# microsoft/MoGe

Measured on NVIDIA H100. Metric: images/sec ViT-L 518px fp16 (MoGe-2 infer), higher is better.
Workload: dtype fp16

## Files before the change

### moge_b200/csrc/common.cuh

```cuda
#pragma once
#include <cuda.h>
#include <cuda_runtime.h>
#include <cuda_fp16.h>
#include <cuda_bf16.h>
#include <stdint.h>
#include <stdio.h>
#include "wgmma.cuh"

namespace mg {

__device__ __forceinline__ uint32_t smem_u32(const void* p) {
    return static_cast<uint32_t>(__cvta_generic_to_shared(p));
}
__device__ __forceinline__ uint32_t lane_id() { return threadIdx.x & 31; }
__device__ __forceinline__ bool elect_one() {
    uint32_t pred;
    asm volatile(
        "{\n\t.reg .pred p;\n\t"
        "elect.sync _|p, 0xffffffff;\n\t"
        "selp.u32 %0, 1, 0, p;\n\t}"
        : "=r"(pred));
    return pred != 0;
}

__device__ __forceinline__ void pdl_launch_dependents() { asm volatile("griddepcontrol.launch_dependents;" ::: "memory"); }
__device__ __forceinline__ void pdl_wait() { asm volatile("griddepcontrol.wait;" ::: "memory"); }
__device__ __forceinline__ void pdl_prologue() {
    pdl_launch_dependents();
    pdl_wait();
}

__device__ __forceinline__ void mbar_init(uint64_t* bar, uint32_t count) {
    asm volatile("mbarrier.init.shared::cta.b64 [%0], %1;" ::"r"(smem_u32(bar)), "r"(count) : "memory");
}
__device__ __forceinline__ void fence_mbar_init() {
    asm volatile("fence.mbarrier_init.release.cluster;" ::: "memory");
}
__device__ __forceinline__ void fence_proxy_async_smem() {
    asm volatile("fence.proxy.async.shared::cta;" ::: "memory");
}
__device__ __forceinline__ void mbar_arrive_expect_tx(uint64_t* bar, uint32_t bytes) {
    asm volatile("mbarrier.arrive.expect_tx.shared::cta.b64 _, [%0], %1;" ::"r"(smem_u32(bar)), "r"(bytes) : "memory");
}
__device__ __forceinline__ void mbar_arrive(uint64_t* bar) {
    asm volatile("mbarrier.arrive.shared::cta.b64 _, [%0];" ::"r"(smem_u32(bar)) : "memory");
}
__device__ __forceinline__ bool mbar_try_wait(uint64_t* bar, uint32_t parity) {
    uint32_t ok;
    asm volatile(
        "{\n\t.reg .pred p;\n\t"
        "mbarrier.try_wait.parity.shared::cta.b64 p, [%1], %2;\n\t"
        "selp.u32 %0, 1, 0, p;\n\t}"
        : "=r"(ok)
        : "r"(smem_u32(bar)), "r"(parity)
        : "memory");
    return ok != 0;
}
#ifndef MG_WATCHDOG_SPINS
#define MG_WATCHDOG_SPINS (1u << 21)
#endif
constexpr int kMaxDynSmem = 232448;
__device__ __forceinline__ void mbar_wait(uint64_t* bar, uint32_t parity) {
    uint32_t spins = 0;
    while (!mbar_try_wait(bar, parity)) {
        if (++spins > MG_WATCHDOG_SPINS) __trap();
    }
}

__device__ __forceinline__ void tma_prefetch_desc(const CUtensorMap* m) {
    asm volatile("prefetch.tensormap [%0];" ::"l"(reinterpret_cast<uint64_t>(m)) : "memory");
}
__device__ __forceinline__ void tma_load_2d(void* dst, const CUtensorMap* m, uint64_t* bar, int c0, int c1) {
    asm volatile(
        "cp.async.bulk.tensor.2d.shared::cluster.global.mbarrier::complete_tx::bytes [%0], [%1, {%3, %4}], [%2];"
        ::"r"(smem_u32(dst)), "l"(reinterpret_cast<uint64_t>(m)), "r"(smem_u32(bar)), "r"(c0), "r"(c1)
        : "memory");
}
__device__ __forceinline__ void tma_load_3d(void* dst, const CUtensorMap* m, uint64_t* bar, int c0, int c1, int c2) {
    asm volatile(
        "cp.async.bulk.tensor.3d.shared::cluster.global.mbarrier::complete_tx::bytes [%0], [%1, {%3, %4, %5}], [%2];"
        ::"r"(smem_u32(dst)), "l"(reinterpret_cast<uint64_t>(m)), "r"(smem_u32(bar)), "r"(c0), "r"(c1), "r"(c2)
        : "memory");
}
__device__ __forceinline__ void tma_load_4d(void* dst, const CUtensorMap* m, uint64_t* bar, int c0, int c1, int c2,
                                            int c3) {
    asm volatile(
        "cp.async.bulk.tensor.4d.shared::cluster.global.mbarrier::complete_tx::bytes [%0], [%1, {%3, %4, %5, %6}], [%2];"
        ::"r"(smem_u32(dst)), "l"(reinterpret_cast<uint64_t>(m)), "r"(smem_u32(bar)), "r"(c0), "r"(c1), "r"(c2),
        "r"(c3)
        : "memory");
}

__device__ __forceinline__ uint64_t make_sdesc_sw128(uint32_t smem_addr, uint32_t lbo_bytes = 16, uint32_t sbo_bytes = 1024) {
    uint64_t d = 0;
    d |= static_cast<uint64_t>((smem_addr & 0x3FFFF) >> 4);
    d |= static_cast<uint64_t>((lbo_bytes >> 4) & 0x3FFF) << 16;
    d |= static_cast<uint64_t>((sbo_bytes >> 4) & 0x3FFF) << 32;
    d |= static_cast<uint64_t>(1) << 62;
    return d;
}
__device__ __forceinline__ void wgmma_fence() { asm volatile("wgmma.fence.sync.aligned;" ::: "memory"); }
__device__ __forceinline__ void wgmma_commit() { asm volatile("wgmma.commit_group.sync.aligned;" ::: "memory"); }
template <int N> __device__ __forceinline__ void wgmma_wait() { asm volatile("wgmma.wait_group.sync.aligned %0;" ::"n"(N) : "memory"); }
template <int N> __device__ __forceinline__ void reg_fence(float (&r)[N]) {
#pragma unroll
    for (int i = 0; i < N; ++i) asm volatile("" : "+f"(r[i])::"memory");
}
__device__ __forceinline__ void named_sync(uint32_t id, uint32_t count) {
    asm volatile("bar.sync %0, %1;" ::"r"(id), "r"(count) : "memory");
}
template <uint32_t R> __device__ __forceinline__ void regs_dec() { asm volatile("setmaxnreg.dec.sync.aligned.u32 %0;" ::"n"(R)); }
template <uint32_t R> __device__ __forceinline__ void regs_inc() { asm volatile("setmaxnreg.inc.sync.aligned.u32 %0;" ::"n"(R)); }

__device__ __forceinline__ float2 ffma2(float2 a, float2 b, float2 c) { return make_float2(fmaf(a.x, b.x, c.x), fmaf(a.y, b.y, c.y)); }
__device__ __forceinline__ float2 fadd2(float2 a, float2 b) { return make_float2(a.x + b.x, a.y + b.y); }
__device__ __forceinline__ float2 fmul2(float2 a, float2 b) { return make_float2(a.x * b.x, a.y * b.y); }

__device__ __forceinline__ float fmax3(float a, float b, float c) {
    float r;
    asm("max.f32 %0, %1, %2, %3;" : "=f"(r) : "f"(a), "f"(b), "f"(c));
    return r;
}
__device__ __forceinline__ float ex2_approx(float x) {
    float r;
    asm("ex2.approx.ftz.f32 %0, %1;" : "=f"(r) : "f"(x));
    return r;
}

template <bool BF16> struct H16;
template <> struct H16<false> {
    using T = __half;
    using T2 = __half2;
    static __device__ __forceinline__ uint32_t pack(float a, float b) {
        __half2 h = __floats2half2_rn(a, b);
        return *reinterpret_cast<uint32_t*>(&h);
    }
    static __device__ __forceinline__ float2 unpack(uint32_t u) {
        return __half22float2(*reinterpret_cast<__half2*>(&u));
    }
    static __device__ __forceinline__ T from_float(float a) { return __float2half_rn(a); }
    static __device__ __forceinline__ float to_float(T a) { return __half2float(a); }
};
template <> struct H16<true> {
    using T = __nv_bfloat16;
    using T2 = __nv_bfloat162;
    static __device__ __forceinline__ uint32_t pack(float a, float b) {
        __nv_bfloat162 h = __floats2bfloat162_rn(a, b);
        return *reinterpret_cast<uint32_t*>(&h);
    }
    static __device__ __forceinline__ float2 unpack(uint32_t u) {
        return __bfloat1622float2(*reinterpret_cast<__nv_bfloat162*>(&u));
    }
    static __device__ __forceinline__ T from_float(float a) { return __float2bfloat16_rn(a); }
    static __device__ __forceinline__ float to_float(T a) { return __bfloat162float(a); }
};

__device__ __forceinline__ float warp_sum(float v) {
#pragma unroll
    for (int o = 16; o > 0; o >>= 1) v += __shfl_xor_sync(0xffffffffu, v, o);
    return v;
}
__device__ __forceinline__ float warp_max(float v) {
#pragma unroll
    for (int o = 16; o > 0; o >>= 1) v = fmaxf(v, __shfl_xor_sync(0xffffffffu, v, o));
    return v;
}

}
```

### moge_b200/csrc/umma_kernel.cuh

```cuda
#pragma once
#include "common.cuh"
#include <type_traits>

namespace mg {

enum : int { AMODE_ROWS = 0, AMODE_TILES = 1 };
enum : int {
    EPI_STORE16 = 0,
    EPI_GELU16 = 1,
    EPI_RESID = 2,
    EPI_PATCH = 3,
    EPI_DEC = 4,
    EPI_HEADOUT = 5,
    EPI_NECKOUT = 6,
};

enum : int { MODE_GEMM = 0, MODE_CONV64 = 1, MODE_CONVH = 2 };
constexpr int TILE_M = 128;
constexpr int TILE_K = 64;
constexpr int TILE_PW = 16;
constexpr int TILE_PH = 8;

struct UmmaParams {
    int M;
    int N;
    int ntaps;
    int kb_main;
    int kb_aux;
    int num_m_tiles, num_n_tiles;
    int B, H, W;
    int tiles_x, tiles_y;
    void* out0;
    void* out1;
    void* out2;
    int accum;
    const float* bias;
    const float* vec1;
    const float* vec2;
    const void* skip;
    int ldo;
    int T;
    int Ho, Wo, Hop, Wop;
    int shuffle;
    int ncomp;
    float su, sv;
    void* x16;
    float2* stats_out;
    const float* ln_rstd;
    int stats_ld;
};

template <int BN, int MODE = MODE_GEMM> struct UmmaCfg {
    static constexpr int kHaloBytes = 160 * 128;
    static constexpr int kABytes = (MODE == MODE_GEMM) ? TILE_M * 128 : kHaloBytes;
    static constexpr int kBBytes = (MODE == MODE_GEMM) ? BN * 128 : (MODE == MODE_CONVH) ? 3 * BN * 128 : 0;
    static constexpr int kStageBytes = kABytes + kBBytes;
    static constexpr int kResidentBytes = (MODE == MODE_CONV64) ? 10 * BN * 128 : 0;
    static constexpr int kChunks = (BN < 32) ? 1 : BN / 32;
    static constexpr int kAccBytes = TILE_M * kChunks * 32 * 4;
    static constexpr int kFixedBytes = kAccBytes + kResidentBytes + 1024  + 256 ;
    static constexpr int kFit = (kMaxDynSmem - kFixedBytes) / kStageBytes;
    static constexpr int kStages = kFit > 8 ? 8 : kFit;
    static constexpr int kEpiWarps = (BN >= 64) ? 8 : 4;
    static constexpr int kThreads = 384;
    static constexpr int kSmemBytes = kStages * kStageBytes + kFixedBytes;
    static constexpr int kColsPerWarp = (kEpiWarps == 8) ? BN / 2 : BN;
    static_assert(kStages >= 2, "umma_kernel: fewer than two ring stages fit beside the accumulator tile");
    static_assert(kSmemBytes <= kMaxDynSmem, "umma_kernel: stage ring + accumulator tile exceed the shared memory of one CTA");
    static_assert((2 * kStages + 1) * 8 <= 256, "umma_kernel: barrier block overflows its 256 bytes");
};

template <int BN>
__device__ __forceinline__ const float4* acc_block(const float4* stg, int quarter, int col) {
    return stg + (quarter * UmmaCfg<BN>::kChunks + (col >> 5)) * 256;
}
template <int BN>
__device__ __forceinline__ void acc_stage(float4* stg, const float* d, int g, int wl, int lane) {
    float* s = reinterpret_cast<float*>(stg);
#pragma unroll
    for (int i = 0; i < BN / 2; i += 2) {
        const int row = 64 * g + 16 * wl + (lane >> 2) + 8 * ((i >> 1) & 1);
        const int col = 8 * (i >> 2) + 2 * (lane & 3);
        const int rl = row & 31, q = (col & 31) >> 2;
        float* blk = s + ((row >> 5) * UmmaCfg<BN>::kChunks + (col >> 5)) * 1024;
        *reinterpret_cast<float2*>(blk + (rl * 8 + (q ^ (rl & 7))) * 4 + (col & 3)) = make_float2(d[i], d[i + 1]);
    }
}
template <int NQ>
__device__ __forceinline__ void acc_row(const float4* blk, int lane, float* v) {
#pragma unroll
    for (int q = 0; q < NQ; ++q) {
        const float4 t = blk[lane * 8 + (q ^ (lane & 7))];
        v[4 * q] = t.x; v[4 * q + 1] = t.y; v[4 * q + 2] = t.z; v[4 * q + 3] = t.w;
    }
}

__device__ __forceinline__ float gelu_erf(float x) {
    const float ax = fabsf(x);
    float q = fmaf(-4.804994387e-04f, ax, 7.133518346e-03f);
    q = fmaf(q, ax, -5.194617063e-02f);
    q = fmaf(q, ax, -4.598676562e-01f);
    q = fmaf(q, ax, -1.150842190e+00f);
    q = fmaf(q, ax, -3.041332639e-05f);
    const float t = ax * ex2_approx(q);
    return fmaf(-0.5f, t, fmaxf(x, 0.0f));
}

__device__ __forceinline__ float2 gelu_erf2(float2 x) {
    const float2 ab = make_float2(fabsf(x.x), fabsf(x.y));
    const float2 ax = ab;
    float2 q = ffma2(make_float2(-4.804994387e-04f, -4.804994387e-04f), ax, make_float2(7.133518346e-03f, 7.133518346e-03f));
    q = ffma2(q, ax, make_float2(-5.194617063e-02f, -5.194617063e-02f));
    q = ffma2(q, ax, make_float2(-4.598676562e-01f, -4.598676562e-01f));
    q = ffma2(q, ax, make_float2(-1.150842190e+00f, -1.150842190e+00f));
    q = ffma2(q, ax, make_float2(-3.041332639e-05f, -3.041332639e-05f));
    const float2 t = fmul2(ab, make_float2(ex2_approx(q.x), ex2_approx(q.y)));
    return ffma2(make_float2(-0.5f, -0.5f), t, make_float2(fmaxf(x.x, 0.0f), fmaxf(x.y, 0.0f)));
}

static __device__ __noinline__ void store_px_border8(uint8_t* base, int b, int Y, int X, int Ho, int Wo, int Hop, int Wop,
                                                 int ld, int c0, uint2 q) {
    uint8_t* centre = base + (((static_cast<size_t>(b) * Hop + Y + 1) * Wop + X + 1) * ld + c0) * 2;
    *reinterpret_cast<uint2*>(centre) = q;
    if (Y != 0 && Y != Ho - 1 && X != 0 && X != Wo - 1) return;
    const int dy0 = (Y == 0) ? -1 : 0, dy1 = (Y == Ho - 1) ? 1 : 0;
    const int dx0 = (X == 0) ? -1 : 0, dx1 = (X == Wo - 1) ? 1 : 0;
    const ptrdiff_t rowp = static_cast<ptrdiff_t>(Wop) * ld * 2, colp = static_cast<ptrdiff_t>(ld) * 2;
    for (int dy = dy0; dy <= dy1; ++dy)
        for (int dx = dx0; dx <= dx1; ++dx)
            if (dy != 0 || dx != 0) *reinterpret_cast<uint2*>(centre + dy * rowp + dx * colp) = q;
}

struct LnRows { float rs[8]; };
__device__ __forceinline__ void ln_load(const UmmaParams& p, int mt, int quarter, int lane, LnRows& r) {
    const int sub = lane >> 3;
#pragma unroll
    for (int i = 0; i < 8; ++i) {
        const long grow = static_cast<long>(mt) * TILE_M + quarter * 32 + 4 * i + sub;
        r.rs[i] = (grow < p.M) ? p.ln_rstd[grow] : 1.f;
    }
}

enum : int { DF_RAW = 1, DF_RELU = 2, DF_SKIP = 4, DF_UV = 8, DF_SHUFFLE = 16 };

static __device__ __noinline__ void store_px_border16(uint8_t* base, int b, int Y, int X, int Ho, int Wo, int Hop, int Wop,
                                                      int ld, int c0, uint4 q) {
    uint8_t* centre = base + (((static_cast<size_t>(b) * Hop + Y + 1) * Wop + X + 1) * ld + c0) * 2;
    const int dy0 = (Y == 0) ? -1 : 0, dy1 = (Y == Ho - 1) ? 1 : 0;
    const int dx0 = (X == 0) ? -1 : 0, dx1 = (X == Wo - 1) ? 1 : 0;
    const ptrdiff_t rowp = static_cast<ptrdiff_t>(Wop) * ld * 2, colp = static_cast<ptrdiff_t>(ld) * 2;
    for (int dy = dy0; dy <= dy1; ++dy)
        for (int dx = dx0; dx <= dx1; ++dx)
            if (dy != 0 || dx != 0) *reinterpret_cast<uint4*>(centre + dy * rowp + dx * colp) = q;
}

template <int BN, int COLS, int AMODE, bool BF16, int DF>
__device__ __forceinline__ void epilogue_dec16(const UmmaParams& p, int mt, int nt, const float4* stg, int quarter, int lane,
                                               int col_begin) {
    using H = H16<BF16>;
    const bool has_raw = (DF < 0) ? (p.out0 != nullptr) : ((DF & DF_RAW) != 0);
    const bool has_relu = (DF < 0) ? (p.out1 != nullptr) : ((DF & DF_RELU) != 0);
    const bool has_skip = (DF < 0) ? (p.skip != nullptr) : ((DF & DF_SKIP) != 0);
    const bool has_uv = (DF < 0) ? (p.vec1 != nullptr) : ((DF & DF_UV) != 0);
    const bool shuffle = (DF < 0) ? (p.shuffle != 0) : ((DF & DF_SHUFFLE) != 0);
    const int sub = lane >> 2;
    const int q8 = lane & 3;
    int tile_b = 0, tile_y0 = 0, tile_x0 = 0;
    if (AMODE == AMODE_TILES) {
        const int per_img = p.tiles_x * p.tiles_y;
        tile_b = mt / per_img;
        const int r = mt % per_img;
        tile_y0 = (r / p.tiles_x) * TILE_PH;
        tile_x0 = (r % p.tiles_x) * TILE_PW;
    }
    bool ok[4];
    int rb[4], ry[4], rx[4], eflags[4];
    size_t roff[4];
    const int sh = shuffle ? 2 : 1;
#pragma unroll
    for (int i = 0; i < 4; ++i) {
        const int rl = quarter * 32 + 8 * i + sub;
        if (AMODE == AMODE_ROWS) {
            const long grow = static_cast<long>(mt) * TILE_M + rl;
            ok[i] = grow < p.M;
            rb[i] = static_cast<int>(grow / p.T);
            const int t = static_cast<int>(grow % p.T);
            ry[i] = t / p.W; rx[i] = t % p.W;
        } else {
            rb[i] = tile_b;
            ry[i] = tile_y0 + rl / TILE_PW;
            rx[i] = tile_x0 + rl % TILE_PW;
            ok[i] = (ry[i] < p.H) && (rx[i] < p.W);
        }
        roff[i] = ((static_cast<size_t>(rb[i]) * p.Hop + sh * ry[i] + 1) * p.Wop + sh * rx[i] + 1) * p.ldo * 2;
        eflags[i] = (ry[i] == 0 ? 1 : 0) | (ry[i] == p.H - 1 ? 2 : 0) | (rx[i] == 0 ? 4 : 0) | (rx[i] == p.W - 1 ? 8 : 0);
    }
    const float inv_wo = 1.0f / static_cast<float>(p.Wo), inv_ho = 1.0f / static_cast<float>(p.Ho);
    bool interior;
    if (AMODE == AMODE_TILES) interior = tile_y0 > 0 && tile_x0 > 0 && tile_y0 + TILE_PH < p.H && tile_x0 + TILE_PW < p.W;
    else interior = false;
    const int ldo_shift = ((p.ldo & (p.ldo - 1)) == 0) ? (31 - __clz(p.ldo)) : -1;
    auto chunk = [&](int c, auto fast_tag) {
        constexpr bool FAST = decltype(fast_tag)::value;
        const float4* scr = acc_block<BN>(stg, quarter, col_begin + c);
        const int col = nt * BN + col_begin + c;
        int co = col + 8 * q8, qd = 0, qmask = 15;
        size_t qoff = 0;
        if (shuffle) {
            qd = (ldo_shift >= 0) ? (col >> ldo_shift) : (col / p.ldo);
            co -= qd * p.ldo;
            qoff = (static_cast<size_t>(qd >> 1) * p.Wop + (qd & 1)) * p.ldo * 2;
            qmask = ((qd >> 1) ? 2 : 1) | ((qd & 1) ? 8 : 4);
        }
        qoff += static_cast<size_t>(co) * 2;
        const float4 b0 = *reinterpret_cast<const float4*>(p.bias + co), b1 = *reinterpret_cast<const float4*>(p.bias + co + 4);
        float4 g0 = make_float4(0.f, 0.f, 0.f, 0.f), g1 = g0, h0 = g0, h1 = g0;
        if (has_uv) {
            g0 = *reinterpret_cast<const float4*>(p.vec1 + co); g1 = *reinterpret_cast<const float4*>(p.vec1 + co + 4);
            h0 = *reinterpret_cast<const float4*>(p.vec2 + co); h1 = *reinterpret_cast<const float4*>(p.vec2 + co + 4);
        }
        uint4 sk[4];
#pragma unroll
        for (int i = 0; i < 4; ++i) {
            sk[i] = make_uint4(0u, 0u, 0u, 0u);
            if (has_skip && (FAST || ok[i])) sk[i] = *reinterpret_cast<const uint4*>(static_cast<const uint8_t*>(p.skip) + roff[i] + qoff);
        }
        uint4 pk_raw[4], pk_relu[4];
        unsigned edge_rows = 0;
#pragma unroll
        for (int i = 0; i < 4; ++i) {
            const int rl = 8 * i + sub;
            float4 a0 = scr[rl * 8 + ((2 * q8) ^ (rl & 7))];
            float4 a1 = scr[rl * 8 + ((2 * q8 + 1) ^ (rl & 7))];
            if (!FAST && !ok[i]) continue;
            a0.x += b0.x; a0.y += b0.y; a0.z += b0.z; a0.w += b0.w;
            a1.x += b1.x; a1.y += b1.y; a1.z += b1.z; a1.w += b1.w;
            if (has_skip) {
                const float2 s0 = H::unpack(sk[i].x), s1 = H::unpack(sk[i].y), s2 = H::unpack(sk[i].z), s3 = H::unpack(sk[i].w);
                a0.x += s0.x; a0.y += s0.y; a0.z += s1.x; a0.w += s1.y;
                a1.x += s2.x; a1.y += s2.y; a1.z += s3.x; a1.w += s3.y;
            }
            if (has_uv) {
                const int X = sh * rx[i] + (qd & 1), Y = sh * ry[i] + (qd >> 1);
                const float uu = p.su * ((2 * X + 1) * inv_wo - 1.0f);
                const float vv = p.sv * ((2 * Y + 1) * inv_ho - 1.0f);
                a0.x += g0.x * uu + h0.x * vv; a0.y += g0.y * uu + h0.y * vv; a0.z += g0.z * uu + h0.z * vv; a0.w += g0.w * uu + h0.w * vv;
                a1.x += g1.x * uu + h1.x * vv; a1.y += g1.y * uu + h1.y * vv; a1.z += g1.z * uu + h1.z * vv; a1.w += g1.w * uu + h1.w * vv;
            }
            if (!FAST && (eflags[i] & qmask) != 0) edge_rows |= 1u << i;
            if (has_raw) {
                pk_raw[i] = make_uint4(H::pack(a0.x, a0.y), H::pack(a0.z, a0.w), H::pack(a1.x, a1.y), H::pack(a1.z, a1.w));
                *reinterpret_cast<uint4*>(static_cast<uint8_t*>(p.out0) + roff[i] + qoff) = pk_raw[i];
            }
            if (has_relu) {
                pk_relu[i] = make_uint4(H::pack(fmaxf(a0.x, 0.f), fmaxf(a0.y, 0.f)), H::pack(fmaxf(a0.z, 0.f), fmaxf(a0.w, 0.f)),
                                        H::pack(fmaxf(a1.x, 0.f), fmaxf(a1.y, 0.f)), H::pack(fmaxf(a1.z, 0.f), fmaxf(a1.w, 0.f)));
                *reinterpret_cast<uint4*>(static_cast<uint8_t*>(p.out1) + roff[i] + qoff) = pk_relu[i];
            }
        }
        if (!FAST && edge_rows != 0) {
#pragma unroll
            for (int i = 0; i < 4; ++i)
                if (edge_rows >> i & 1) {
                    const int X = sh * rx[i] + (qd & 1), Y = sh * ry[i] + (qd >> 1);
                    if (has_raw) store_px_border16(static_cast<uint8_t*>(p.out0), rb[i], Y, X, p.Ho, p.Wo, p.Hop, p.Wop, p.ldo, co, pk_raw[i]);
                    if (has_relu) store_px_border16(static_cast<uint8_t*>(p.out1), rb[i], Y, X, p.Ho, p.Wo, p.Hop, p.Wop, p.ldo, co, pk_relu[i]);
                }
        }
    };
    if (interior) {
#pragma unroll 1
        for (int c = 0; c < COLS; c += 32) chunk(c, std::true_type{});
    } else {
#pragma unroll 1
        for (int c = 0; c < COLS; c += 32) chunk(c, std::false_type{});
    }
}



template <int BN, int COLS, int AMODE, int EPI, bool BF16, int DF = -1>
__device__ __forceinline__ void epilogue_tile(const UmmaParams& p, int mt, int nt, const float4* stg, int quarter,
                                              int lane, int col_begin, bool ln_rows_on = false, LnRows lnr = LnRows{}) {
    using H = H16<BF16>;
    const bool has_raw = (DF < 0) ? (p.out0 != nullptr) : ((DF & DF_RAW) != 0);
    const bool has_relu = (DF < 0) ? (p.out1 != nullptr) : ((DF & DF_RELU) != 0);
    const bool has_skip = (DF < 0) ? (p.skip != nullptr) : ((DF & DF_SKIP) != 0);
    const bool has_uv = (DF < 0) ? (p.vec1 != nullptr) : ((DF & DF_UV) != 0);
    const bool shuffle = (DF < 0) ? (p.shuffle != 0) : ((DF & DF_SHUFFLE) != 0);
    if (EPI == EPI_DEC) {
        epilogue_dec16<BN, COLS, AMODE, BF16, DF>(p, mt, nt, stg, quarter, lane, col_begin);
        return;
    }
    const int row = quarter * 32 + lane;
    const int sub = lane >> 3;
    const int q4 = lane & 7;
    if (EPI == EPI_HEADOUT) {
        const int per_img = p.tiles_x * p.tiles_y;
        const int b = mt / per_img;
        const int r = mt % per_img;
        const int py = (r / p.tiles_x) * TILE_PH + row / TILE_PW;
        const int px = (r % p.tiles_x) * TILE_PW + row % TILE_PW;
        const bool valid = (py < p.H) && (px < p.W);
        float v[16];
        acc_row<4>(acc_block<BN>(stg, quarter, 0), lane, v);
        if (valid) {
#pragma unroll
            for (int ph = 0; ph < 4; ++ph) {
                const int Y = 2 * py + (ph >> 1), X = 2 * px + (ph & 1);
                float o[3];
#pragma unroll
                for (int k = 0; k < 3; ++k) o[k] = (k < p.ncomp) ? v[ph * p.ncomp + k] + p.bias[k] : 0.f;
                if (p.vec1 != nullptr) {
                    const uint4* src = reinterpret_cast<const uint4*>(
                        static_cast<const uint8_t*>(p.skip) + ((static_cast<size_t>(b) * p.Hop + Y + 1) * p.Wop + X + 1) * 64);
#pragma unroll
                    for (int q = 0; q < 4; ++q) {
                        const uint4 u = src[q];
                        const uint32_t w[4] = {u.x, u.y, u.z, u.w};
#pragma unroll
                        for (int e = 0; e < 4; ++e) {
                            const float2 f = H::unpack(w[e]);
                            const int c = q * 8 + e * 2;
#pragma unroll
                            for (int k = 0; k < 3; ++k)
                                if (k < p.ncomp) o[k] += p.vec1[k * 32 + c] * f.x + p.vec1[k * 32 + c + 1] * f.y;
                        }
                    }
                }
                const size_t pix = (static_cast<size_t>(b) * p.Ho + Y) * p.Wo + X;
                if (p.accum) {
                    if (p.ncomp == 1) o[0] += static_cast<const float*>(p.out0)[pix];
                    else { const float4 t = static_cast<const float4*>(p.out0)[pix]; o[0] += t.x; o[1] += t.y; o[2] += t.z; }
                }
                if (p.ncomp == 1) static_cast<float*>(p.out0)[pix] = o[0];
                else static_cast<float4*>(p.out0)[pix] = make_float4(o[0], o[1], o[2], 0.f);
            }
        }
        __syncwarp();
    } else if (EPI == EPI_NECKOUT) {
        const int per_img = p.tiles_x * p.tiles_y;
        const int b = mt / per_img;
        const int r = mt % per_img;
        const int py = (r / p.tiles_x) * TILE_PH + row / TILE_PW;
        const int px = (r % p.tiles_x) * TILE_PW + row % TILE_PW;
        const bool valid = (py < p.H) && (px < p.W);
        float v[32];
        acc_row<8>(acc_block<BN>(stg, quarter, 0), lane, v);
        if (valid) {
            float b8[8], gu[8], gv[8];
#pragma unroll
            for (int k = 0; k < 8; ++k) { b8[k] = p.bias[k]; gu[k] = p.vec1[k]; gv[k] = p.vec2[k]; }
            const float inv_wo = 1.0f / static_cast<float>(p.Wo), inv_ho = 1.0f / static_cast<float>(p.Ho);
#pragma unroll
            for (int ph = 0; ph < 4; ++ph) {
                const int Y = 2 * py + (ph >> 1), X = 2 * px + (ph & 1);
                const float uu = p.su * ((2 * X + 1) * inv_wo - 1.0f);
                const float vv = p.sv * ((2 * Y + 1) * inv_ho - 1.0f);
                float o[8];
#pragma unroll
                for (int k = 0; k < 8; ++k) o[k] = v[ph * 8 + k] + b8[k] + gu[k] * uu + gv[k] * vv;
                const size_t pix = (static_cast<size_t>(b) * p.Ho + Y) * p.Wo + X;
                if (p.out0) static_cast<float4*>(p.out0)[pix] = make_float4(o[0], o[1], o[2], 0.f);
                if (p.out1) static_cast<float4*>(p.out1)[pix] = make_float4(o[3], o[4], o[5], 0.f);
                if (p.out2) static_cast<float*>(p.out2)[pix] = o[6];
            }
        }
        __syncwarp();
    } else {
        int tile_b = 0, tile_y0 = 0, tile_x0 = 0;
        if (AMODE == AMODE_TILES) {
            const int per_img = p.tiles_x * p.tiles_y;
            tile_b = mt / per_img;
            const int r = mt % per_img;
            tile_y0 = (r / p.tiles_x) * TILE_PH;
            tile_x0 = (r % p.tiles_x) * TILE_PW;
        }
        bool ok[8];
        int rb[8], ry[8], rx[8];
        size_t roff[8];
        int eflags[8];
        int xrow[8];
#pragma unroll
        for (int i = 0; i < 8; ++i) {
            const int rl = quarter * 32 + 4 * i + sub;
            rb[i] = 0; ry[i] = 0; rx[i] = 0; roff[i] = 0; eflags[i] = 0; xrow[i] = 0;
            if (AMODE == AMODE_ROWS) {
                const long grow = static_cast<long>(mt) * TILE_M + rl;
                ok[i] = grow < p.M;
                xrow[i] = static_cast<int>(grow);
                roff[i] = static_cast<size_t>(grow) * p.ldo;
                if (EPI == EPI_DEC || EPI == EPI_PATCH) {
                    rb[i] = static_cast<int>(grow / p.T);
                    const int t = static_cast<int>(grow % p.T);
                    ry[i] = t / p.W; rx[i] = t % p.W;
                    if (EPI == EPI_PATCH) {
                        xrow[i] = rb[i] * (p.T + 1) + 1 + t;
                        roff[i] = static_cast<size_t>(xrow[i]) * p.ldo;
                    }
                }
            } else {
                rb[i] = tile_b;
                ry[i] = tile_y0 + rl / TILE_PW;
                rx[i] = tile_x0 + rl % TILE_PW;
                ok[i] = (ry[i] < p.H) && (rx[i] < p.W);
            }
            if (EPI == EPI_DEC) {
                const int sh = shuffle ? 2 : 1;
                roff[i] = ((static_cast<size_t>(rb[i]) * p.Hop + sh * ry[i] + 1) * p.Wop + sh * rx[i] + 1) * p.ldo * 2;
                eflags[i] = (ry[i] == 0 ? 1 : 0) | (ry[i] == p.H - 1 ? 2 : 0) | (rx[i] == 0 ? 4 : 0) | (rx[i] == p.W - 1 ? 8 : 0);
            }
        }
        const float inv_wo = 1.0f / static_cast<float>(p.Wo), inv_ho = 1.0f / static_cast<float>(p.Ho);
        constexpr bool LN_CONS = (EPI == EPI_STORE16 || EPI == EPI_GELU16) && AMODE == AMODE_ROWS;
        constexpr bool LN_PROD = (EPI == EPI_RESID || EPI == EPI_PATCH) && AMODE == AMODE_ROWS;
        const bool ln_on = LN_CONS && ln_rows_on;
        const bool x16_on = LN_PROD && p.x16 != nullptr;
        float ln_rs[8], st1[8], st2[8];
#pragma unroll
        for (int i = 0; i < 8; ++i) { ln_rs[i] = ln_on ? lnr.rs[i] : 1.f; st1[i] = 0.f; st2[i] = 0.f; }
        const bool full_tile = (AMODE == AMODE_ROWS) && (static_cast<long>(mt) + 1) * TILE_M <= static_cast<long>(p.M);
        auto chunk = [&](int c, auto full_tag) {
            constexpr bool FULL = decltype(full_tag)::value;
            const int col = nt * BN + col_begin + c;
            int co = col + 4 * q4;
            float4 pre[8];
            const float4* scr = acc_block<BN>(stg, quarter, col_begin + c);
            int qd = 0;
            size_t qoff = 0;
            int qmask = 15;
            if (EPI == EPI_DEC && shuffle) {
                qd = col / p.ldo;
                co -= qd * p.ldo;
                qoff = (static_cast<size_t>(qd >> 1) * p.Wop + (qd & 1)) * p.ldo * 2;
                qmask = ((qd >> 1) ? 2 : 1) | ((qd & 1) ? 8 : 4);
            }
            if (EPI == EPI_DEC) qoff += static_cast<size_t>(co) * 2;
            float4 bias4 = make_float4(0.f, 0.f, 0.f, 0.f), g4 = bias4, h4 = bias4;
            if (EPI != EPI_PATCH) bias4 = *reinterpret_cast<const float4*>(p.bias + co);
            if (EPI == EPI_RESID) g4 = *reinterpret_cast<const float4*>(p.vec1 + co);
            if (EPI == EPI_DEC && has_uv) {
                g4 = *reinterpret_cast<const float4*>(p.vec1 + co);
                h4 = *reinterpret_cast<const float4*>(p.vec2 + co);
            }
            int sY[8], sX[8];
#pragma unroll
            for (int i = 0; i < 8; ++i) {
                pre[i] = make_float4(0.f, 0.f, 0.f, 0.f);
                sY[i] = ry[i]; sX[i] = rx[i];
                if (EPI == EPI_DEC && shuffle) { sY[i] = 2 * ry[i] + (qd >> 1); sX[i] = 2 * rx[i] + (qd & 1); }
                if (!FULL && !ok[i]) continue;
                if (EPI == EPI_RESID) {
                    pre[i] = *reinterpret_cast<const float4*>(static_cast<const float*>(p.out0) + roff[i] + co);
                } else if (EPI == EPI_PATCH) {
                    const int t = ry[i] * p.W + rx[i];
                    pre[i] = *reinterpret_cast<const float4*>(p.vec1 + static_cast<size_t>(t) * p.ldo + co);
                } else if (EPI == EPI_DEC && has_skip) {
                    const uint2 u = *reinterpret_cast<const uint2*>(static_cast<const uint8_t*>(p.skip) + roff[i] + qoff);
                    const float2 f0 = H::unpack(u.x), f1 = H::unpack(u.y);
                    pre[i] = make_float4(f0.x, f0.y, f1.x, f1.y);
                }
            }
            uint2 pk_raw[8], pk_relu[8];
            unsigned edge_rows = 0;
#pragma unroll
            for (int i = 0; i < 8; ++i) {
                const int rl = 4 * i + sub;
                float4 a = scr[rl * 8 + (q4 ^ (rl & 7))];
                if (!FULL && !ok[i]) continue;
                if (EPI == EPI_STORE16 || EPI == EPI_GELU16) {
                    float2 a01, a23;
                    if (ln_on) {
                        a01 = make_float2(fmaf(ln_rs[i], a.x, bias4.x), fmaf(ln_rs[i], a.y, bias4.y));
                        a23 = make_float2(fmaf(ln_rs[i], a.z, bias4.z), fmaf(ln_rs[i], a.w, bias4.w));
                    } else {
                        a01 = make_float2(a.x + bias4.x, a.y + bias4.y);
                        a23 = make_float2(a.z + bias4.z, a.w + bias4.w);
                    }
                    if (EPI == EPI_GELU16) { a01 = gelu_erf2(a01); a23 = gelu_erf2(a23); }
                    uint2 pk;
                    pk.x = H::pack(a01.x, a01.y); pk.y = H::pack(a23.x, a23.y);
                    *reinterpret_cast<uint2*>(static_cast<typename H::T*>(p.out0) + roff[i] + co) = pk;
                } else if (EPI == EPI_RESID) {
                    float4 x = pre[i];
                    x.x += g4.x * (a.x + bias4.x); x.y += g4.y * (a.y + bias4.y);
                    x.z += g4.z * (a.z + bias4.z); x.w += g4.w * (a.w + bias4.w);
                    *reinterpret_cast<float4*>(static_cast<float*>(p.out0) + roff[i] + co) = x;
                    const float2 x01 = make_float2(x.x, x.y), x23 = make_float2(x.z, x.w);
                    if (x16_on) {
                        uint2 pk;
                        pk.x = H::pack(x01.x, x01.y); pk.y = H::pack(x23.x, x23.y);
                        *reinterpret_cast<uint2*>(static_cast<typename H::T*>(p.x16) + roff[i] + co) = pk;
                        const float2 f0 = H::unpack(pk.x), f1 = H::unpack(pk.y);
                        const float2 s1 = fadd2(f0, f1), s2 = ffma2(f0, f0, fmul2(f1, f1));
                        st1[i] += s1.x + s1.y;
                        st2[i] += s2.x + s2.y;
                    }
                } else if (EPI == EPI_PATCH) {
                    const float4 x = make_float4(a.x + pre[i].x, a.y + pre[i].y, a.z + pre[i].z, a.w + pre[i].w);
                    *reinterpret_cast<float4*>(static_cast<float*>(p.out0) + roff[i] + co) = x;
                    if (x16_on) {
                        uint2 pk;
                        pk.x = H::pack(x.x, x.y); pk.y = H::pack(x.z, x.w);
                        *reinterpret_cast<uint2*>(static_cast<typename H::T*>(p.x16) + roff[i] + co) = pk;
                        const float2 f0 = H::unpack(pk.x), f1 = H::unpack(pk.y);
                        const float2 s1 = fadd2(f0, f1), s2 = ffma2(f0, f0, fmul2(f1, f1));
                        st1[i] += s1.x + s1.y;
                        st2[i] += s2.x + s2.y;
                    }
                } else if (EPI == EPI_DEC) {
                    a.x += bias4.x + pre[i].x; a.y += bias4.y + pre[i].y; a.z += bias4.z + pre[i].z; a.w += bias4.w + pre[i].w;
                    if (has_uv) {
                        const float uu = p.su * ((2 * sX[i] + 1) * inv_wo - 1.0f);
                        const float vv = p.sv * ((2 * sY[i] + 1) * inv_ho - 1.0f);
                        a.x += g4.x * uu + h4.x * vv; a.y += g4.y * uu + h4.y * vv;
                        a.z += g4.z * uu + h4.z * vv; a.w += g4.w * uu + h4.w * vv;
                    }
                    if ((eflags[i] & qmask) != 0) edge_rows |= 1u << i;
                    if (has_raw) {
                        pk_raw[i].x = H::pack(a.x, a.y); pk_raw[i].y = H::pack(a.z, a.w);
                        *reinterpret_cast<uint2*>(static_cast<uint8_t*>(p.out0) + roff[i] + qoff) = pk_raw[i];
                    }
                    if (has_relu) {
                        pk_relu[i].x = H::pack(fmaxf(a.x, 0.f), fmaxf(a.y, 0.f)); pk_relu[i].y = H::pack(fmaxf(a.z, 0.f), fmaxf(a.w, 0.f));
                        *reinterpret_cast<uint2*>(static_cast<uint8_t*>(p.out1) + roff[i] + qoff) = pk_relu[i];
                    }
                }
            }
            if (EPI == EPI_DEC && edge_rows != 0) {
#pragma unroll
                for (int i = 0; i < 8; ++i)
                    if (edge_rows >> i & 1) {
                        if (has_raw) store_px_border8(static_cast<uint8_t*>(p.out0), rb[i], sY[i], sX[i], p.Ho, p.Wo, p.Hop, p.Wop, p.ldo, co, pk_raw[i]);
                        if (has_relu) store_px_border8(static_cast<uint8_t*>(p.out1), rb[i], sY[i], sX[i], p.Ho, p.Wo, p.Hop, p.Wop, p.ldo, co, pk_relu[i]);
                    }
            }
            __syncwarp();
        };
        if (full_tile) {
#pragma unroll 1
            for (int c = 0; c < COLS; c += 32) chunk(c, std::true_type{});
        } else {
#pragma unroll 1
            for (int c = 0; c < COLS; c += 32) chunk(c, std::false_type{});
        }
        if (x16_on) {
            const int part = (nt * BN + col_begin) / COLS;
#pragma unroll
            for (int i = 0; i < 8; ++i) {
                float a = st1[i], b = st2[i];
#pragma unroll
                for (int o = 1; o < 8; o <<= 1) { a += __shfl_xor_sync(0xffffffffu, a, o); b += __shfl_xor_sync(0xffffffffu, b, o); }
                if (q4 == 0 && ok[i]) p.stats_out[static_cast<size_t>(xrow[i]) * p.stats_ld + part] = make_float2(a, b);
            }
        }
    }
}

template <int BN, int MODE, int AMODE, int EPI, bool BF16, int DF = -1>
__global__ void __launch_bounds__(384, 1)
umma_kernel(const __grid_constant__ CUtensorMap mapA, const __grid_constant__ CUtensorMap mapAux,
            const __grid_constant__ CUtensorMap mapB, const UmmaParams p) {
    pdl_launch_dependents();
    using Cfg = UmmaCfg<BN, MODE>;
    constexpr int S = Cfg::kStages;
    extern __shared__ uint8_t smem_raw[];
    uint8_t* smem = smem_raw + ((1024u - (smem_u32(smem_raw) & 1023u)) & 1023u);
    float4* stg = reinterpret_cast<float4*>(smem + S * Cfg::kStageBytes);
    uint8_t* sW = smem + S * Cfg::kStageBytes + Cfg::kAccBytes;
    uint64_t* full = reinterpret_cast<uint64_t*>(sW + Cfg::kResidentBytes);
    uint64_t* empty = full + S;
    uint64_t* wfull = empty + S;

    const int warp = threadIdx.x >> 5;
    const int lane = threadIdx.x & 31;
    const int total_tiles = p.num_m_tiles * p.num_n_tiles;
    const int kb_taps = p.ntaps * p.kb_main;
    const int nstage = (MODE == MODE_GEMM) ? kb_taps + p.kb_aux : (MODE == MODE_CONV64) ? 3 + p.kb_aux : 3 * p.kb_main + p.kb_aux;

    if (threadIdx.x == 0) {
        tma_prefetch_desc(&mapA);
        tma_prefetch_desc(&mapB);
        if (p.kb_aux) tma_prefetch_desc(&mapAux);
        for (int s = 0; s < S; ++s) { mbar_init(&full[s], 1); mbar_init(&empty[s], 8); }
        mbar_init(wfull, 1);
        fence_mbar_init();
    }
    __syncthreads();
    pdl_wait();

    if (warp < 4) {
        regs_dec<40>();
        if (warp != 0) return;
        if (MODE == MODE_CONV64) {
            const int nblk = 9 + p.kb_aux;
            const int nt = static_cast<int>(blockIdx.x) % p.num_n_tiles;
            if (elect_one()) {
                mbar_arrive_expect_tx(wfull, nblk * BN * 128);
                for (int t = 0; t < nblk; ++t) tma_load_2d(sW + t * BN * 128, &mapB, wfull, t * TILE_K, nt * BN);
            }
            __syncwarp();
        }
        int s = 0; uint32_t ph = 0;
        for (int tile = blockIdx.x; tile < total_tiles; tile += gridDim.x) {
            const int mt = tile / p.num_n_tiles, nt = tile % p.num_n_tiles;
            int b = 0, x0 = 0, y0 = 0;
            if (AMODE == AMODE_TILES) {
                const int per_img = p.tiles_x * p.tiles_y;
                b = mt / per_img;
                const int r = mt % per_img;
                y0 = (r / p.tiles_x) * TILE_PH;
                x0 = (r % p.tiles_x) * TILE_PW;
            }
            for (int i = 0; i < nstage; ++i) {
                mbar_wait(&empty[s], ph ^ 1);
                uint8_t* sa = smem + s * Cfg::kStageBytes;
                uint8_t* sb = sa + Cfg::kABytes;
                if (elect_one()) {
                    if (MODE == MODE_GEMM) {
                        mbar_arrive_expect_tx(&full[s], Cfg::kStageBytes);
                        if (AMODE == AMODE_ROWS) {
                            tma_load_2d(sa, &mapA, &full[s], i * TILE_K, mt * TILE_M);
                        } else if (i < kb_taps) {
                            const int tap = i / p.kb_main, c = i % p.kb_main;
                            const int tx = (p.ntaps == 9) ? tap % 3 : 1, ty = (p.ntaps == 9) ? tap / 3 : 1;
                            tma_load_4d(sa, &mapA, &full[s], c * TILE_K, x0 + tx, y0 + ty, b);
                        } else {
                            tma_load_4d(sa, &mapAux, &full[s], (i - kb_taps) * TILE_K, x0 + 1, y0 + 1, b);
                        }
                        tma_load_2d(sb, &mapB, &full[s], i * TILE_K, nt * BN);
                    } else if (MODE == MODE_CONV64) {
                        if (i < 3) {
                            mbar_arrive_expect_tx(&full[s], Cfg::kHaloBytes);
                            tma_load_4d(sa, &mapA, &full[s], 0, x0 + i, y0, b);
                        } else {
                            mbar_arrive_expect_tx(&full[s], TILE_M * 128);
                            tma_load_4d(sa, &mapAux, &full[s], 0, x0 + 1, y0 + 1, b);
                        }
                    } else {
                        const bool aux = i >= 3 * p.kb_main;
                        if (!aux) {
                            const int c = i / 3, dx = i % 3;
                            mbar_arrive_expect_tx(&full[s], Cfg::kHaloBytes + 3 * BN * 128);
                            tma_load_4d(sa, &mapA, &full[s], c * TILE_K, x0 + dx, y0, b);
                            for (int dy = 0; dy < 3; ++dy)
                                tma_load_2d(sb + dy * BN * 128, &mapB, &full[s], ((dy * 3 + dx) * p.kb_main + c) * TILE_K, nt * BN);
                        } else {
                            const int c = i - 3 * p.kb_main;
                            mbar_arrive_expect_tx(&full[s], TILE_M * 128 + BN * 128);
                            tma_load_4d(sa, &mapAux, &full[s], c * TILE_K, x0 + 1, y0 + 1, b);
                            tma_load_2d(sb, &mapB, &full[s], (9 * p.kb_main + c) * TILE_K, nt * BN);
                        }
                    }
                }
                __syncwarp();
                if (++s == S) { s = 0; ph ^= 1; }
            }
        }
    } else {
        regs_inc<232>();
        const int g = (warp - 4) >> 2;
        const int wl = warp & 3;
        const int ew = warp - 4;
        const int quarter = ew & 3;
        const int col_begin = (Cfg::kEpiWarps == 8) ? (ew >> 2) * (BN / 2) : 0;
        const uint32_t a_off = static_cast<uint32_t>(g) * 64 * 128;
        if (MODE == MODE_CONV64) mbar_wait(wfull, 0);
        const uint32_t w0 = smem_u32(sW);
        LnRows lnr{}, lnn{};
        const bool ln_on = AMODE == AMODE_ROWS && (EPI == EPI_STORE16 || EPI == EPI_GELU16) && p.ln_rstd != nullptr;
        if (ln_on && static_cast<int>(blockIdx.x) < total_tiles) ln_load(p, static_cast<int>(blockIdx.x) / p.num_n_tiles, quarter, lane, lnn);
        int s = 0; uint32_t ph = 0;
        for (int tile = blockIdx.x; tile < total_tiles; tile += gridDim.x) {
            const int mt = tile / p.num_n_tiles, nt = tile % p.num_n_tiles;
            if (ln_on) {
                lnr = lnn;
                const int nxt = tile + static_cast<int>(gridDim.x);
                if (nxt < total_tiles) ln_load(p, nxt / p.num_n_tiles, quarter, lane, lnn);
            }
            float acc[BN / 2];
#pragma unroll
            for (int j = 0; j < BN / 2; ++j) acc[j] = 0.f;
            int prev = -1;
            for (int i = 0; i < nstage; ++i) {
                mbar_wait(&full[s], ph);
                const uint32_t sa = smem_u32(smem + s * Cfg::kStageBytes) + a_off;
                const uint32_t sb = smem_u32(smem + s * Cfg::kStageBytes + Cfg::kABytes);
                wgmma_fence();
                auto mma64 = [&](uint32_t a, uint32_t bb) {
                    const uint64_t ad = make_sdesc_sw128(a), bd = make_sdesc_sw128(bb);
#pragma unroll
                    for (int k = 0; k < TILE_K / 16; ++k) Wgmma<BN, BF16>::ss(acc, ad + 2 * k, bd + 2 * k, 1u);
                };
                if (MODE == MODE_GEMM) {
                    mma64(sa, sb);
                } else if (MODE == MODE_CONV64) {
                    if (i < 3) {
#pragma unroll
                        for (int dy = 0; dy < 3; ++dy) mma64(sa + dy * TILE_PW * 128, w0 + (dy * 3 + i) * BN * 128);
                    } else {
                        mma64(sa, w0 + 9 * BN * 128);
                    }
                } else {
                    if (i < 3 * p.kb_main) {
#pragma unroll
                        for (int dy = 0; dy < 3; ++dy) mma64(sa + dy * TILE_PW * 128, sb + dy * BN * 128);
                    } else {
                        mma64(sa, sb);
                    }
                }
                wgmma_commit();
                wgmma_wait<1>();
                reg_fence(acc);
                if (prev >= 0 && lane == 0) mbar_arrive(&empty[prev]);
                prev = s;
                if (++s == S) { s = 0; ph ^= 1; }
            }
            wgmma_wait<0>();
            reg_fence(acc);
            if (prev >= 0 && lane == 0) mbar_arrive(&empty[prev]);
            named_sync(1, 256);
            acc_stage<BN>(stg, acc, g, wl, lane);
            named_sync(1, 256);
            if (ew < Cfg::kEpiWarps)
                epilogue_tile<BN, Cfg::kColsPerWarp, AMODE, EPI, BF16, DF>(p, mt, nt, stg, quarter, lane, col_begin, ln_on, lnr);
        }
    }
}

}
```

Before: 204.8.

## Ping-pong two consumer warpgroups over alternate tiles to overlap MMA with epilogue

Each consumer warpgroup now takes alternate tiles and computes the full 128-row tile on its own, issuing two wgmma per k-step into a doubled accumulator. Named barriers pass turns between the groups, so one group's epilogue runs while the other issues MMAs. The per-stage empty barrier count drops to 4 warps to match. The aim is to hide epilogue time behind tensor core work, at the cost of doubled accumulator registers per thread, more barrier coordination, and a shared staging buffer that is serialised between the groups.

```diff
diff --git a/moge_b200/csrc/common.cuh b/moge_b200/csrc/common.cuh
--- a/moge_b200/csrc/common.cuh
+++ b/moge_b200/csrc/common.cuh
@@ -109,6 +109,9 @@
 __device__ __forceinline__ void named_sync(uint32_t id, uint32_t count) {
     asm volatile("bar.sync %0, %1;" ::"r"(id), "r"(count) : "memory");
 }
+__device__ __forceinline__ void named_arrive(uint32_t id, uint32_t count) {
+    asm volatile("bar.arrive %0, %1;" ::"r"(id), "r"(count) : "memory");
+}
 template <uint32_t R> __device__ __forceinline__ void regs_dec() { asm volatile("setmaxnreg.dec.sync.aligned.u32 %0;" ::"n"(R)); }
 template <uint32_t R> __device__ __forceinline__ void regs_inc() { asm volatile("setmaxnreg.inc.sync.aligned.u32 %0;" ::"n"(R)); }
 
diff --git a/moge_b200/csrc/umma_kernel.cuh b/moge_b200/csrc/umma_kernel.cuh
--- a/moge_b200/csrc/umma_kernel.cuh
+++ b/moge_b200/csrc/umma_kernel.cuh
@@ -61,10 +61,9 @@
     static constexpr int kFixedBytes = kAccBytes + kResidentBytes + 1024  + 256 ;
     static constexpr int kFit = (kMaxDynSmem - kFixedBytes) / kStageBytes;
     static constexpr int kStages = kFit > 8 ? 8 : kFit;
-    static constexpr int kEpiWarps = (BN >= 64) ? 8 : 4;
     static constexpr int kThreads = 384;
     static constexpr int kSmemBytes = kStages * kStageBytes + kFixedBytes;
-    static constexpr int kColsPerWarp = (kEpiWarps == 8) ? BN / 2 : BN;
+    static constexpr int kPassCols = (BN >= 64) ? BN / 2 : BN;
     static_assert(kStages >= 2, "umma_kernel: fewer than two ring stages fit beside the accumulator tile");
     static_assert(kSmemBytes <= kMaxDynSmem, "umma_kernel: stage ring + accumulator tile exceed the shared memory of one CTA");
     static_assert((2 * kStages + 1) * 8 <= 256, "umma_kernel: barrier block overflows its 256 bytes");
@@ -75,15 +74,19 @@
     return stg + (quarter * UmmaCfg<BN>::kChunks + (col >> 5)) * 256;
 }
 template <int BN>
-__device__ __forceinline__ void acc_stage(float4* stg, const float* d, int g, int wl, int lane) {
+__device__ __forceinline__ void acc_stage(float4* stg, const float* d, int wl, int lane) {
     float* s = reinterpret_cast<float*>(stg);
 #pragma unroll
-    for (int i = 0; i < BN / 2; i += 2) {
-        const int row = 64 * g + 16 * wl + (lane >> 2) + 8 * ((i >> 1) & 1);
-        const int col = 8 * (i >> 2) + 2 * (lane & 3);
-        const int rl = row & 31, q = (col & 31) >> 2;
-        float* blk = s + ((row >> 5) * UmmaCfg<BN>::kChunks + (col >> 5)) * 1024;
-        *reinterpret_cast<float2*>(blk + (rl * 8 + (q ^ (rl & 7))) * 4 + (col & 3)) = make_float2(d[i], d[i + 1]);
+    for (int m = 0; m < 2; ++m) {
+#pragma unroll
+        for (int i = 0; i < BN / 2; i += 2) {
+            const int row = 64 * m + 16 * wl + (lane >> 2) + 8 * ((i >> 1) & 1);
+            const int col = 8 * (i >> 2) + 2 * (lane & 3);
+            const int rl = row & 31, q = (col & 31) >> 2;
+            float* blk = s + ((row >> 5) * UmmaCfg<BN>::kChunks + (col >> 5)) * 1024;
+            *reinterpret_cast<float2*>(blk + (rl * 8 + (q ^ (rl & 7))) * 4 + (col & 3)) =
+                make_float2(d[m * (BN / 2) + i], d[m * (BN / 2) + i + 1]);
+        }
     }
 }
 template <int NQ>
@@ -582,7 +585,7 @@
         tma_prefetch_desc(&mapA);
         tma_prefetch_desc(&mapB);
         if (p.kb_aux) tma_prefetch_desc(&mapAux);
-        for (int s = 0; s < S; ++s) { mbar_init(&full[s], 1); mbar_init(&empty[s], 8); }
+        for (int s = 0; s < S; ++s) { mbar_init(&full[s], 1); mbar_init(&empty[s], 4); }
         mbar_init(wfull, 1);
         fence_mbar_init();
     }
@@ -659,38 +662,38 @@
         }
     } else {
         regs_inc<232>();
-        const int g = (warp - 4) >> 2;
+        const int g = __shfl_sync(0xffffffffu, (warp - 4) >> 2, 0);
         const int wl = warp & 3;
-        const int ew = warp - 4;
-        const int quarter = ew & 3;
-        const int col_begin = (Cfg::kEpiWarps == 8) ? (ew >> 2) * (BN / 2) : 0;
-        const uint32_t a_off = static_cast<uint32_t>(g) * 64 * 128;
         if (MODE == MODE_CONV64) mbar_wait(wfull, 0);
         const uint32_t w0 = smem_u32(sW);
-        LnRows lnr{}, lnn{};
+        LnRows lnr{};
         const bool ln_on = AMODE == AMODE_ROWS && (EPI == EPI_STORE16 || EPI == EPI_GELU16) && p.ln_rstd != nullptr;
-        if (ln_on && static_cast<int>(blockIdx.x) < total_tiles) ln_load(p, static_cast<int>(blockIdx.x) / p.num_n_tiles, quarter, lane, lnn);
-        int s = 0; uint32_t ph = 0;
-        for (int tile = blockIdx.x; tile < total_tiles; tile += gridDim.x) {
+        const int first = static_cast<int>(blockIdx.x) + g * static_cast<int>(gridDim.x);
+        const int step = 2 * static_cast<int>(gridDim.x);
+        if (ln_on && first < total_tiles) ln_load(p, first / p.num_n_tiles, wl, lane, lnr);
+        constexpr uint32_t kTurnBar = 2, kEpiBar = 4, kStgBar = 6;
+        int pos = g * nstage;
+        for (int tile = first; tile < total_tiles; tile += step, pos += 2 * nstage) {
             const int mt = tile / p.num_n_tiles, nt = tile % p.num_n_tiles;
-            if (ln_on) {
-                lnr = lnn;
-                const int nxt = tile + static_cast<int>(gridDim.x);
-                if (nxt < total_tiles) ln_load(p, nxt / p.num_n_tiles, quarter, lane, lnn);
-            }
-            float acc[BN / 2];
-#pragma unroll
-            for (int j = 0; j < BN / 2; ++j) acc[j] = 0.f;
+            if (tile != static_cast<int>(blockIdx.x)) named_sync(kTurnBar + g, 256);
+            int s = pos % S;
+            uint32_t ph = (pos / S) & 1;
+            float acc[BN];
+#pragma unroll
+            for (int j = 0; j < BN; ++j) acc[j] = 0.f;
             int prev = -1;
             for (int i = 0; i < nstage; ++i) {
                 mbar_wait(&full[s], ph);
-                const uint32_t sa = smem_u32(smem + s * Cfg::kStageBytes) + a_off;
+                const uint32_t sa = smem_u32(smem + s * Cfg::kStageBytes);
                 const uint32_t sb = smem_u32(smem + s * Cfg::kStageBytes + Cfg::kABytes);
                 wgmma_fence();
                 auto mma64 = [&](uint32_t a, uint32_t bb) {
-                    const uint64_t ad = make_sdesc_sw128(a), bd = make_sdesc_sw128(bb);
-#pragma unroll
-                    for (int k = 0; k < TILE_K / 16; ++k) Wgmma<BN, BF16>::ss(acc, ad + 2 * k, bd + 2 * k, 1u);
+                    const uint64_t ad0 = make_sdesc_sw128(a), ad1 = make_sdesc_sw128(a + 64 * 128), bd = make_sdesc_sw128(bb);
+#pragma unroll
+                    for (int k = 0; k < TILE_K / 16; ++k) {
+                        Wgmma<BN, BF16>::ss(acc, ad0 + 2 * k, bd + 2 * k, 1u);
+                        Wgmma<BN, BF16>::ss(acc + BN / 2, ad1 + 2 * k, bd + 2 * k, 1u);
+                    }
                 };
                 if (MODE == MODE_GEMM) {
                     mma64(sa, sb);
@@ -716,16 +719,21 @@
                 prev = s;
                 if (++s == S) { s = 0; ph ^= 1; }
             }
+            const bool next = tile + static_cast<int>(gridDim.x) < total_tiles;
+            if (next) named_arrive(kTurnBar + (g ^ 1), 256);
             wgmma_wait<0>();
             reg_fence(acc);
             if (prev >= 0 && lane == 0) mbar_arrive(&empty[prev]);
-            named_sync(1, 256);
-            acc_stage<BN>(stg, acc, g, wl, lane);
-            named_sync(1, 256);
-            if (ew < Cfg::kEpiWarps)
-                epilogue_tile<BN, Cfg::kColsPerWarp, AMODE, EPI, BF16, DF>(p, mt, nt, stg, quarter, lane, col_begin, ln_on, lnr);
-        }
-    }
-}
-
-}
+            if (tile != static_cast<int>(blockIdx.x)) named_sync(kEpiBar + g, 256);
+            acc_stage<BN>(stg, acc, wl, lane);
+            named_sync(kStgBar + g, 128);
+#pragma unroll 1
+            for (int c = 0; c < BN; c += Cfg::kPassCols)
+                epilogue_tile<BN, Cfg::kPassCols, AMODE, EPI, BF16, DF>(p, mt, nt, stg, wl, lane, c, ln_on, lnr);
+            if (next) named_arrive(kEpiBar + (g ^ 1), 256);
+            if (ln_on && tile + step < total_tiles) ln_load(p, (tile + step) / p.num_n_tiles, wl, lane, lnr);
+        }
+    }
+}
+
+}
```

New measurement: 214.7, median of 6. 1.05x the previous value.
